# puzzlepaint/surfelmeshing

Hardware: AMD Instinct MI355X
Metric: RGB-D frames/s integrated @640x480, 5M live surfels; achieved HBM GB/s (higher is better)
Workload: dtype f32; 1 GPU; C2: synthetic room stream 640x480, raw depth + colour frames resident in HBM, full preprocessing + Integrate per frame, 4912850 live surfels (6250000 slots), steady-state re-traversal; max_surfel_count=6250000, streams=1, parallelism=1 independent stream per GPU

## Files before the change

### surfelmeshing_amd/csrc/smx_recon.hip

```cpp
#include <math.h>
#include <cmath>
#include <stdlib.h>
#include <string.h>

#include <algorithm>
#include <atomic>
#include <vector>

#include "smx_recon_state.hpp"
#include "smx_mesh.hpp"
#include <hip/hip_ext.h>

using namespace smx;

namespace {

struct FrameCtx {
  Mat34 L;
  Mat34 G;
  float fx, fy, cx, cy;
  Unproj up;
  float inv_depth_scaling;
  float sensor_noise_factor;
  float cos_normal_compat;
// ... 462 lines not shown
    return __builtin_amdgcn_readfirstlane(longest) * kSubLists;
  }
  ent = 0; cntv = 0;
  return (n_slots_scan + kBlock - 1) / kBlock;
}
template <bool kUseList>
__device__ __forceinline__ bool vis_entry(uint32_t ent, uint32_t c, uint32_t cntv, uint32_t n_slots_scan, uint32_t lane, uint32_t& i) {
  if (kUseList) {
    const uint32_t k = __builtin_amdgcn_readfirstlane(c % kSubLists);
    const uint32_t len = (uint32_t)__builtin_amdgcn_readlane((int)cntv, (int)k);
    i = ent;
    return (c / kSubLists) * (uint32_t)kBlock + lane < len;
  }
  i = c * kBlock + lane;
  return i < n_slots_scan;
}

struct PairRec { uint32_t i, code; Vec3 g, l, gn; float r2; };
__device__ __forceinline__ PairRec fetch_pair(const Surfels& S, const FrameCtx& c, uint32_t i, uint32_t code) {
  const float4 p4 = *S.group(kGroupP, i), n4 = *S.group(kGroupN, i);
  PairRec r;
  r.i = i; r.code = code;
  r.g = Vec3{p4.x, p4.y, p4.z};
  r.l = mul(c.L, r.g);
  r.gn = Vec3{n4.x, n4.y, n4.z};
  r.r2 = n4.w;
  return r;
}
struct TileLds {
  int zmin[kTilePx];
  uint32_t sup[kTilePx], cnt[kTilePx], confl[kTilePx];
  unsigned long long sum[kTilePx];
  float2 nrm[kTilePx];
  uint16_t depth[kTilePx];
};
__device__ __forceinline__ void assoc_stage(TileLds& t, const FrameCtx& c, const PairRec& r) {
  if (!(r.code & kPairActive)) return;
  const uint32_t k = r.code & 255u;
  const float measurement_depth = c.inv_depth_scaling * (float)t.depth[k];
  if (measurement_depth <= 0) return;
  const float first = __int_as_float(t.zmin[k]);
  if (first < (1 - c.sensor_noise_factor) * measurement_depth) {
    if (first == r.l.z) atomicMin(&t.confl[k], 0x80000000u | r.i);
    return;
  }
  const float occlusion_depth = (1 + c.sensor_noise_factor) * measurement_depth;
  if (r.l.z > occlusion_depth) return;
  const float surfel_distance = sqrtf(r.l.x * r.l.x + r.l.y * r.l.y + r.l.z * r.l.z);
  const Vec3 ln = rotate(c.L, r.gn);
  const float dot_angle = (1.0f / surfel_distance) * (r.l.x * ln.x + r.l.y * ln.y + r.l.z * ln.z);
  if (dot_angle > 0) return;
  if (measurement_depth < r.l.z) {
    const float2 n = t.nrm[k];
    const float nz = meas_normal_z(n.x, n.y);
    const float d = ln.x * n.x + ln.y * n.y + ln.z * nz;
    if (d < c.cos_normal_compat) return;
  }
  if (r.r2 <= 0) return;
  atomicMin(&t.sup[k], r.i);
  atomicAdd(&t.cnt[k], 1u);
  atomicAdd(&t.sum[k], (unsigned long long)q_from_float(r.l.z));
}
__device__ __forceinline__ uint32_t merge_candidate(TileLds& t, const FrameCtx& c, const PairRec& r) {
  if (r.code & kPairSecond) return kInvalid;
  if (!(r.r2 >= 0)) return kInvalid;
  const uint32_t k = r.code & 255u;
// ... 28 lines not shown
  const float dx = r.g.x - sp4.x, dy = r.g.y - sp4.y, dz = r.g.z - sp4.z;
  const float d2 = dx * dx + dy * dy + dz * dz;
  const float kDist = 0.5f * (0.25f * 0.25f);
  if (d2 > kDist * (r.r2 + other_r2)) return;
  const float dot_angle = r.gn.x * sn4.x + r.gn.y * sn4.y + r.gn.z * sn4.z;
  if (dot_angle < 0.93969f) return;
  merge_flag[r.i] = 1;
}
__device__ __forceinline__ void merge_stage(TileLds& t, const Surfels& S, const FrameCtx& c, const PairRec& r,
                                            uint8_t* __restrict__ merge_flag) {
  const uint32_t s = merge_candidate(t, c, r);
  if (s == kInvalid) return;
  const float4 sp4 = *S.group(kGroupP, s), sn4 = *S.group(kGroupN, s);
  keep(sp4); keep(sn4);
  merge_decide(r, sp4, sn4, merge_flag);
}

constexpr int kPairCache = 4;
template <class F>
__device__ __forceinline__ void for_uncached_pairs(const Surfels& S, const FrameCtx& c, const TileBins& tb, uint32_t tile,
                                                   uint32_t n_binned, bool overflowed, uint32_t n_ovf, F f) {
  for (uint32_t k = kPairCache * kTilePx + threadIdx.x; k < n_binned; k += kTilePx) {
    const uint2 pr = tb.pairs[(size_t)tile * tb.cap + k];
    f(fetch_pair(S, c, pr.x, pr.y));
  }
  if (overflowed)
    for (uint32_t e = threadIdx.x; e < n_ovf; e += kTilePx) {
      const uint4 o = tb.ovf[e];
      if (o.x == tile) f(fetch_pair(S, c, o.y, o.z));
    }
}

__global__ void __launch_bounds__(kTilePx)
k_assoc_tiles(Surfels S, FrameCtx c, Scratch sc, Img<const uint16_t> depth, Img<const float2> normals, TileBins tb,
              uint32_t* __restrict__ next_ovf_count, uint8_t* __restrict__ merge_flag, DevState* st,
              const uint8_t* __restrict__ seg_act, uint32_t nseg, uint32_t* __restrict__ direction_out, uint32_t* __restrict__ seg_work_count,
              unsigned long long* stamps, const unsigned long long* __restrict__ ts_ring, volatile unsigned long long* ts_host,
              unsigned long long ts_seq) {
  SMX_SET_WAVE_PRIO();
  __shared__ TileLds t;
  __shared__ uint32_t order_wave_tot[kTilePx / 64];
  ts_begin(c.ts, kTsTilesBegin);
  if (blockIdx.x == 0 && threadIdx.x == 64 && ts_host && ts_seq > 2) {
    const unsigned long long q = ts_seq - 2;
    const unsigned long long* src = ts_ring + (size_t)(q % kTsRing) * kTsWords;
    volatile unsigned long long* dst = ts_host + (size_t)(q % kTsRing) * kTsWords;
    unsigned long long w[kTsWords];
#pragma unroll
    for (int k = 0; k < kTsWords; ++k) w[k] = src[k];
    if (w[kTsSeq] == q) {
      unsigned long long check = q ^ kTsCheckSalt;
#pragma unroll
      for (int k = 1; k < kTsSeqTail; ++k) check ^= w[k];
      dst[kTsSeq] = q;
#pragma unroll
      for (int k = 1; k < kTsSeqTail; ++k) dst[k] = w[k];
      dst[kTsSeqTail] = check;
    }
  }
  if (blockIdx.x == 0) {
    const uint32_t n_used = min(nseg, (st->surfel_count + (uint32_t)kSeg - 1u) / (uint32_t)kSeg);
    choose_segment_direction(seg_act, n_used, direction_out, order_wave_tot);
    __syncthreads();
  }
  SMX_STAMP(stamps, 0);
  const uint32_t tile = blockIdx.x, lane = threadIdx.x;
  const int x = (int)(tile % (uint32_t)tb.tiles_x) * kTileW + (int)(lane % kTileW);
  const int y = (int)(tile / (uint32_t)tb.tiles_x) * kTileH + (int)(lane / kTileW);
  const bool in_image = x < c.W && y < c.H;
  const uint32_t n_total = tb.count[tile * kCountStride];
  const uint32_t n_ovf = *tb.ovf_count;
  const uint32_t n_binned = n_total < tb.cap ? n_total : tb.cap;
  const bool overflowed = n_total > tb.cap;
  uint2 pr[kPairCache];
  bool have[kPairCache];
#pragma unroll
  for (int q = 0; q < kPairCache; ++q) {
    const uint32_t k = q * kTilePx + lane;
    have[q] = k < n_binned;
    pr[q] = tb.pairs[(size_t)tile * tb.cap + (have[q] ? k : 0u)];
  }
#pragma unroll
  for (int q = 0; q < kPairCache; ++q) { keep(pr[q].x); keep(pr[q].y); if (!have[q]) pr[q] = make_uint2(0u, 0u); }
  const uint16_t own_depth = in_image ? depth(y, x) : (uint16_t)0;
  const float2 own_normal = in_image ? normals(y, x) : make_float2(0.f, 0.f);
  PairRec rec[kPairCache];
#pragma unroll
  for (int q = 0; q < kPairCache; ++q) rec[q] = fetch_pair(S, c, pr[q].x, pr[q].y);
  t.zmin[lane] = 0x7F800000;
  t.sup[lane] = kInvalid; t.cnt[lane] = 0; t.confl[lane] = kInvalid; t.sum[lane] = 0;
  t.depth[lane] = own_depth; t.nrm[lane] = own_normal;
  __syncthreads();
  SMX_STAMP(stamps, 1);
  auto zmin_stage = [&](const PairRec& r) { if (r.code & kPairActive) atomicMin(&t.zmin[r.code & 255u], __float_as_int(r.l.z)); };
#pragma unroll
  for (int q = 0; q < kPairCache; ++q) if (have[q]) zmin_stage(rec[q]);
  for_uncached_pairs(S, c, tb, tile, n_binned, overflowed, n_ovf, zmin_stage);
  __syncthreads();
  SMX_STAMP(stamps, 2);
  if (lane == 0) {
    tb.count[tile * kCountStride] = 0;
    if (tile == 0) { *next_ovf_count = 0; seg_work_count[0] = 0; seg_work_count[1] = 0; }
    if (c.stats) {
      atomicAdd(&st->n_pairs, n_total);
      atomicMax(&st->max_tile_pairs, n_total);
      if (tile == 0) st->n_overflow_pairs = n_ovf;
    }
  }
#pragma unroll
  for (int q = 0; q < kPairCache; ++q) if (have[q]) assoc_stage(t, c, rec[q]);
  for_uncached_pairs(S, c, tb, tile, n_binned, overflowed, n_ovf, [&](const PairRec& r) { assoc_stage(t, c, r); });
  __syncthreads();
  SMX_STAMP(stamps, 3);
  uint32_t cand[kPairCache];
  float4 cp4[kPairCache], cn4[kPairCache];
#pragma unroll
  for (int q = 0; q < kPairCache; ++q) cand[q] = have[q] ? merge_candidate(t, c, rec[q]) : kInvalid;
#pragma unroll
  for (int q = 0; q < kPairCache; ++q) {
    const uint32_t g = cand[q] == kInvalid ? 0u : cand[q];
    cp4[q] = *S.group(kGroupP, g); cn4[q] = *S.group(kGroupN, g);
  }
#pragma unroll
  for (int q = 0; q < kPairCache; ++q) { keep(cp4[q]); keep(cn4[q]); }
#pragma unroll
  for (int q = 0; q < kPairCache; ++q) if (cand[q] != kInvalid) merge_decide(rec[q], cp4[q], cn4[q], merge_flag);
  for_uncached_pairs(S, c, tb, tile, n_binned, overflowed, n_ovf, [&](const PairRec& r) { merge_stage(t, S, c, r, merge_flag); });
  __syncthreads();
  SMX_STAMP(stamps, 4);
  if (in_image) {
    const size_t k = (size_t)y * c.W + x;
    sc.first_depth[k] = __int_as_float(t.zmin[lane]);
    sc.supporting[k] = t.sup[lane];
    sc.counts[k] = t.cnt[lane];
    sc.depth_sums[k] = (long long)t.sum[lane];
    sc.confl_key[k] = t.confl[lane];
  }
  SMX_STAMP(stamps, 5);
  ts_end(c.ts, kTsTilesEnd, blockIdx.x, gridDim.x);
}

__device__ __forceinline__ float depth_sum_avg(const Scratch& sc, size_t k) {
  return q_to_float(sc.depth_sums[k]) / (float)sc.counts[k];
}

__global__ void __launch_bounds__(kBlock)
k_blend_start(float ds, Img<uint16_t> depth, Scratch sc, BlendBufs b, int W, int H, unsigned long long* ts) {
  ts_end(ts, kTsBlendEnd, blockIdx.y * gridDim.x + blockIdx.x, gridDim.x * gridDim.y);
  const int x = blockIdx.x * 64 + (threadIdx.x & 63);
  const int y = blockIdx.y * 4 + (threadIdx.x >> 6);
  if (!(x >= 1 && y >= 1 && x < W - 1 && y < H - 1)) return;
  const size_t k = (size_t)y * W + x;
  const uint16_t own = depth(y, x);
  if (own == 0 || sc.supporting[k] == kInvalid) return;
  bool measurement_border = false, surfel_border = false;
  for (int wy = y - 1; wy <= y + 1; ++wy)
    for (int wx = x - 1; wx <= x + 1; ++wx) {
      if (depth(wy, wx) == 0) measurement_border = true;
      else if (sc.supporting[(size_t)wy * W + wx] == kInvalid) surfel_border = true;
    }
  if (surfel_border) {
    b.new_distance_map[k] = 1;
    const float avg = depth_sum_avg(sc, k);
    b.new_deltas[k] = avg - (float)own / ds;
  }
  if (measurement_border) {
    b.distance_map[k] = 1;
    const float avg = depth_sum_avg(sc, k);
    b.deltas[k] = avg - (float)own / ds;
// ... 318 lines not shown
  for (int off = 1; off < 64; off <<= 1) {
    const uint32_t t = __shfl_up(incl, off);
    if (lane >= (uint32_t)off) incl += t;
  }
  if (lane == 63) wave_tot[wave] = incl;
  __syncthreads();
  uint32_t wave_off = 0, total = 0;
#pragma unroll
  for (int w = 0; w < kBlock / 64; ++w) {
    if ((uint32_t)w < wave) wave_off += wave_tot[w];
    total += wave_tot[w];
  }
  uint32_t run = wave_off + incl - mine;
#pragma unroll
  for (int j = 0; j < kScanPxPerThread; ++j) {
    const int k = k0 + j;
    if (k < P) local_rank[k] = run;
    run += f[j];
  }
  if (threadIdx.x == 0) {
    block_sums[block] = total;
    if (block == 0) st->create_base_next = st->surfel_count;
  }
}

struct FrameIn {
  Img<const uint16_t> depth; Img<const float2> normals; Img<const float> radius; Img<const uchar3> color;
};

struct PixelIn {
  uint16_t depth; float first; uint32_t key; uint32_t count; float2 nxy; uchar3 col; float radius;
};
__device__ __forceinline__ PixelIn load_pixel(const FrameCtx& c, const Scratch& sc, const FrameIn& in, int x, int y) {
  const size_t k = (size_t)y * c.W + x;
  PixelIn p;
  p.depth = in.depth(y, x); p.first = sc.first_depth[k]; p.key = sc.confl_key[k]; p.count = sc.counts[k];
  p.nxy = in.normals(y, x); p.col = in.color(y, x); p.radius = in.radius(y, x);
  return p;
}

__device__ __forceinline__ void keep(const PixelIn& p) {
  keep((uint32_t)p.depth); keep(p.first); keep(p.key); keep(p.count); keep(p.nxy); keep(p.radius);
  keep((uint32_t)p.col.x | ((uint32_t)p.col.y << 8) | ((uint32_t)p.col.z << 16));
}

struct SurfelRegs {
  float4 P;
  float4 N;
  float4 C;
  bool dirty;
  bool replaced;
  Vec3 new_smooth;
};

__device__ __forceinline__ void integrate_or_conflict(SurfelRegs& R, const FrameCtx& c, const PixelIn& px,
                                                      bool integrate, int x, int y,
                                                      const Vec3& cam, uint32_t i, DevState* st) {
  if (!integrate) return;
  const float measurement_depth = c.inv_depth_scaling * (float)px.depth;
  if (measurement_depth <= 0) return;
  bool conflicting = false;
  const float first = px.first;
  if (first < (1 - c.sensor_noise_factor) * measurement_depth) {
    if (first == cam.z) {
      const uint32_t key = px.key;
      if (key != kInvalid && (key & 0x7FFFFFFFu) == i) conflicting = true;
    }
    integrate = false;
  }
  if (!integrate && !conflicting) return;
// ... 259 lines not shown
      if (j < per && bidx < n_scan_blocks) { block_offsets[bidx] = run; run += v[j]; }
    }
  } else {
    for (int j = 0; j < per; ++j) {
      const int bidx = threadIdx.x * per + j;
      if (bidx < n_scan_blocks) mine += block_sums[bidx];
    }
    uint32_t run = block_excl_scan(mine, wave_tot, total);
    for (int j = 0; j < per; ++j) {
      const int bidx = threadIdx.x * per + j;
      if (bidx < n_scan_blocks) { block_offsets[bidx] = run; run += block_sums[bidx]; }
    }
  }
  __syncthreads();
  const uint32_t room = max_surfels - base;
  const uint32_t created = total < room ? total : room;
  if (block == 0) {
    for (int bidx = threadIdx.x; bidx < n_scan_blocks; bidx += kBlock) block_offsets_out[bidx] = block_offsets[bidx];
    if (threadIdx.x == 0) {
      st->create_base = base;
      st->new_count = created;
      st->capacity_clamped = (total > room) ? 1u : 0u;
      st->surfel_count = base + created;
    }
  }
  const int kDX[4] = {-1, 1, 0, 0}, kDY[4] = {0, 0, -1, 1};
  const int W = c.W, H = c.H, P = W * H;
  for (int k = block * kBlock + threadIdx.x; k < P; k += n_blocks * kBlock) {
    const uint32_t rank = block_offsets[k / kScanPxPerBlock] + ranks[k];
    if (flags[k] != 1 || rank >= created) continue;
    const int y = k / W, x = k - y * W;
    const uint32_t i = base + rank;
    const uint32_t depth_u = in.depth(y, x);
    const float2 nxy = in.normals(y, x);
    const uchar3 col = in.color(y, x);
    const float r2 = in.radius(y, x);
    uint32_t nsup[4], nflag[4], nrank_local[4], ndepth_u[4];
    int kks[4];
#pragma unroll
    for (int d = 0; d < 4; ++d) {
      const int yy = min(max(y + kDY[d], 0), H - 1), xx = min(max(x + kDX[d], 0), W - 1);
      kks[d] = yy * W + xx;
      nsup[d] = sc.supporting[kks[d]];
      nflag[d] = flags[kks[d]];
      nrank_local[d] = ranks[kks[d]];
      ndepth_u[d] = in.depth(yy, xx);
    }
    keep(depth_u); keep(nxy); keep(r2); keep((uint32_t)col.x | ((uint32_t)col.y << 8) | ((uint32_t)col.z << 16));
#pragma unroll
    for (int d = 0; d < 4; ++d) { keep(nsup[d]); keep(nflag[d]); keep(nrank_local[d]); keep(ndepth_u[d]); }
    float4 np4[4], ns4[4];
#pragma unroll
    for (int d = 0; d < 4; ++d) {
      const uint32_t gidx = nsup[d] != kInvalid ? nsup[d] : base;
      np4[d] = *S.group(kGroupP, gidx);
      ns4[d] = *S.group(kGroupS, gidx);
    }
#pragma unroll
    for (int d = 0; d < 4; ++d) { keep(np4[d]); keep(ns4[d]); }
    const float depth = c.inv_depth_scaling * (float)depth_u;
    const Vec3 lp = {depth * (c.up.fx_inv * (float)x + c.up.cx_inv), depth * (c.up.fy_inv * (float)y + c.up.cy_inv), depth};
    const Vec3 gp = mul(c.G, lp);
    const Vec3 mn = {nxy.x, nxy.y, meas_normal_z(nxy.x, nxy.y)};
    const Vec3 gn = rotate(c.G, mn);
    Vec3 sum = {0, 0, 0};
    int count_plus_1 = 1;
    uint32_t nbs[4];
#pragma unroll
    for (int d = 0; d < 4; ++d) {
      uint32_t nb = nsup[d];
      if (nb != kInvalid) {
        const float dx = np4[d].x - gp.x, dy = np4[d].y - gp.y, dz = np4[d].z - gp.z;
        const float d2 = dx * dx + dy * dy + dz * dz;
        if (d2 > c.rf2 * r2) nb = kInvalid;
        else {
          sum.x = sum.x + ns4[d].x; sum.y = sum.y + ns4[d].y; sum.z = sum.z + ns4[d].z;
          ++count_plus_1;
        }
      } else if (nflag[d] == 1) {
        const uint32_t nrank = block_offsets[kks[d] / kScanPxPerBlock] + nrank_local[d];
        if (nrank < created) {
// ... 679 lines not shown
  }
  if (threadIdx.x == 0) *total_out = carry;
}
__global__ void __launch_bounds__(kBlock)
k_delta_gather(Surfels S, uint8_t* __restrict__ dirty8, const uint32_t* __restrict__ seg_offset, float* __restrict__ out,
               uint32_t total, const DevState* st) {
  __shared__ uint32_t wave_tot[kBlock / 64];
  const uint32_t N = st->surfel_count, i0 = blockIdx.x * kSeg + threadIdx.x * 4;
  uint32_t bits = 0;
  if (i0 < N) {
    const uchar4 d = *reinterpret_cast<const uchar4*>(&dirty8[i0]);
    bits = (d.x != 0 ? 1u : 0u) | ((i0 + 1 < N && d.y != 0) ? 2u : 0u) | ((i0 + 2 < N && d.z != 0) ? 4u : 0u) |
           ((i0 + 3 < N && d.w != 0) ? 8u : 0u);
    if (bits) *reinterpret_cast<uchar4*>(&dirty8[i0]) = make_uchar4(0, 0, 0, 0);
  }
  uint32_t seg_total;
  uint32_t off = seg_offset[blockIdx.x] + block_excl_scan((uint32_t)__popc(bits), wave_tot, seg_total);
  const int want[8] = {kSmoothX, kSmoothY, kSmoothZ, kRadiusSq, kNormalX, kNormalY, kNormalZ, kLastUpdateStamp};
#pragma unroll
  for (int j = 0; j < 4; ++j)
    if (bits & (1u << j)) {
      const uint32_t i = i0 + j;
      out[off] = __uint_as_float(i);
#pragma unroll
      for (int k = 0; k < 8; ++k) out[(size_t)(k + 1) * total + off] = S.f(want[k], i);
      ++off;
    }
}

__global__ void __launch_bounds__(kBlock)
k_decode_conflicting(const uint32_t* __restrict__ key, uint32_t* __restrict__ out, int P) {
  const int k = blockIdx.x * kBlock + threadIdx.x;
  if (k < P) out[k] = (key[k] == kInvalid) ? kInvalid : (key[k] & 0x7FFFFFFFu);
}

__global__ void __launch_bounds__(kBlock)
k_global_ranks(const uint32_t* __restrict__ local_rank, const uint32_t* __restrict__ block_offsets,
               uint32_t* __restrict__ out, int P) {
  const int k = blockIdx.x * kBlock + threadIdx.x;
  if (k < P) out[k] = block_offsets[k / kScanPxPerBlock] + local_rank[k];
}

}

enum : int {
  kSlotScanVisible = 0, kSlotAssocTiles, kSlotBlend, kSlotIntegrate,
  kSlotUpdateNeighbors, kSlotNeighborScan,
  kSlotRegAccumulate, kSlotRegStep,
  kSlotRegUpdate,
  kSlotCull,
  kSlotEmpty,
  kSlotCount
};
static const char* const kSlotNames[kSlotCount] = {
  "scan_visible", "assoc_tiles", "blend", "integrate+new_flags", "update_neighbors+create",
  "neighbor_scan", "reg_accumulate", "reg_step", "reg_update", "cull_segments", "empty_slot"};

struct SlotTimer {
  smx_recon r; hipStream_t st; int slot; bool kev, prof, by_launch;
  SlotTimer(smx_recon r_, hipStream_t st_, int slot_, bool launch_carries = false) : r(r_), st(st_), slot(slot_) {
    kev = (r->timing_enabled & 2) != 0;
    prof = (r->prof_slot == slot) && r->prof_ev && r->prof_n < r->prof_cap;
    by_launch = prof && launch_carries;
    if (kev) (void)hipEventRecord(r->kev[2 * slot], st);
    if (prof && !by_launch) (void)hipEventRecord(r->prof_ev[2 * r->prof_n], st);
  }
// ... 162 lines not shown
  r->L.rec_chunks.stride = (uint32_t)(div_up(r->nsegB, kSubLists) + 8192);
  SMX_TRY(r->mem.alloc(&r->L.rec_chunks.desc, (size_t)kSubLists * r->L.rec_chunks.stride, true));
  SMX_TRY(r->mem.alloc(&r->L.rec_chunks.count, (size_t)kSubLists * kCountStride, true));
  static_assert(kSegAcc == kSegB && kAccCount < kCountStride, "pass B lists the edge kernel's segments by its own segment numbers");
  r->L.acc_chunks.stride = r->L.rec_chunks.stride;
  r->L.acc_chunks.count = r->L.rec_chunks.count + kAccCount;
  SMX_TRY(r->mem.alloc(&r->L.acc_chunks.desc, (size_t)kSubLists * r->L.acc_chunks.stride, true));
  SMX_TRY(r->mem.alloc(&r->flags_buf[0], (size_t)r->nsegB * kSegB, true));
  SMX_TRY(r->mem.alloc(&r->flags_buf[1], (size_t)r->nsegB * kSegB, true));
  r->L.flags8 = r->flags_buf[0];
  r->L.hot_shift = 10;
  while ((((size_t)r->nseg * kSeg) >> r->L.hot_shift) + 1 > (size_t)kMaxHotGroups) ++r->L.hot_shift;
  r->L.n_hot_groups = (uint32_t)((((size_t)r->nseg * kSeg) >> r->L.hot_shift) + 1);
  SMX_TRY(r->mem.alloc(&r->L.hot_epoch, (size_t)r->L.n_hot_groups + 64, true));
  SMX_TRY(r->mem.alloc(&r->L.seg_targets, (size_t)r->nsegB * kBlockB, true));
  r->L.epoch = 128;
  r->hot_filter_enabled = 1;
  r->fuse_edges = kFuseEdgesDefault;
  r->hot_holdoff = 3;
  SMX_TRY(r->mem.alloc(&r->merge_flag, r->S.pitch, true));
  SMX_TRY(r->mem.alloc(&r->gate_count, 32, true));
  r->gate_expected = 0;
  constexpr int kHandoverModeDefault = 1;
  r->handover_mode = kHandoverModeDefault;
  {
    const char* cc = getenv("ROCPROF_COUNTER_COLLECTION");
    if (cc && cc[0] && strcmp(cc, "0") != 0) r->handover_mode = 0;
  }
  SMX_TRY(r->mem.alloc(&r->L.act_list, (size_t)r->nsegB * kSegB, true));
  SMX_TRY(r->mem.alloc(&r->sc.supporting, P, true));
  SMX_TRY(r->mem.alloc(&r->sc.counts, P, true));
  SMX_TRY(r->mem.alloc(&r->sc.depth_sums, P, true));
  SMX_TRY(r->mem.alloc(&r->sc.confl_key, P, true));
  SMX_TRY(r->mem.alloc(&r->sc.first_depth, P, true));
  for (int k = 0; k < 2; ++k) {
    SMX_TRY(r->mem.alloc(&r->vis_count_set[k], (size_t)kSubLists * kCountStride, true));
    SMX_TRY(r->mem.alloc(&r->ovf_count_set[k], 1, true));
  }
  r->L.vis_chunks.count = r->vis_count_set[0];
  r->tb.tiles_x = div_up(width, kTileW);
  r->tb.n_tiles = (uint32_t)(r->tb.tiles_x * div_up(height, kTileH));
  r->tb.cap = r->bin_cap_full = kTileBinCap;
  SMX_TRY(r->mem.alloc(&r->tb.pairs, (size_t)r->tb.n_tiles * kTileBinCap, false));
  SMX_TRY(r->mem.alloc(&r->tb.count, (size_t)r->tb.n_tiles * kCountStride, true));
  SMX_TRY(r->mem.alloc(&r->tb.ovf, 2 * (size_t)r->S.pitch + 64, false));
  r->tb.ovf_count = r->ovf_count_set[0];
#ifdef SMX_STAMPS
  SMX_TRY(r->mem.alloc(&r->stamps, (size_t)3 * 16 * 8192, true));
#endif
  SMX_TRY(r->mem.alloc(&r->blended_depth, P, true));
  SMX_TRY(r->mem.alloc(&r->bb.distance_map, P, true));
  SMX_TRY(r->mem.alloc(&r->bb.new_distance_map, P, true));
  SMX_TRY(r->mem.alloc(&r->bb.deltas, P, true));
  SMX_TRY(r->mem.alloc(&r->bb.new_deltas, P, true));
  SMX_TRY(r->mem.alloc(&r->new_flags, P, true));
  SMX_TRY(r->mem.alloc(&r->new_ranks, P, true));
  SMX_TRY(r->mem.alloc(&r->tmp_u32, P, true));
  r->n_scan_blocks = div_up((long long)P, kScanPxPerBlock);
  SMX_TRY(r->mem.alloc(&r->block_sums, (size_t)r->n_scan_blocks, true));
  SMX_TRY(r->mem.alloc(&r->block_offsets, (size_t)r->n_scan_blocks, true));
  SMX_TRY(r->mem.alloc(&r->st, 1, true));
  SMX_TRY(r->mem.alloc(&r->ts_ring, (size_t)kTsRing * kTsWords, true));
  SMX_TRY(r->mem.alloc_host(&r->ts_host, (size_t)kTsRing * kTsWords, false));
  SMX_TRY(r->mem.alloc_host(&r->ts_mapped, (size_t)kTsRing * kTsWords, true));
  memset(const_cast<unsigned long long*>(r->ts_mapped), 0, sizeof(unsigned long long) * kTsRing * kTsWords);
  SMX_TRY(hip_rc(hipHostGetDevicePointer(reinterpret_cast<void**>(&r->ts_mapped_dev), const_cast<unsigned long long*>(r->ts_mapped), 0), "hipHostGetDevicePointer"));
  SMX_TRY(hip_rc(hipDeviceGetAttribute(&r->wall_khz, hipDeviceAttributeWallClockRate, device), "hipDeviceGetAttribute"));
// ... 189 lines not shown
  const Img<uint16_t> depth_rw = as_img<uint16_t>(depth);

  const uint8_t* flags_prev = r->L.flags8;
  r->L.flags8 = (r->L.flags8 == r->flags_buf[0]) ? r->flags_buf[1] : r->flags_buf[0];
  r->L.epoch = (r->L.epoch + 1u) & 255u;
  if (r->hot_holdoff > 0) --r->hot_holdoff;
  const bool pipelined = r->overlap_enabled != 0;
  const hipStream_t sF = st;
  const hipStream_t sR = pipelined ? r->reg_stream : st;
  const bool split = pipelined && (r->debug_skip & 16) != 0;
  if (r->reg_pending && r->last_stream != st) SMX_CALL(join_regularizer(r, st));
  r->last_stream = st;
  if (r->stats_enabled) hipLaunchKernelGGL(k_reset_frame_stats, dim3(1), dim3(1), 0, sF, r->st, 1);
  if (tm) SMX_HIP(hipEventRecord(r->ev[0], sF));
  r->L.descending = *reinterpret_cast<volatile uint32_t*>(r->dir_host);
  r->sc_cur ^= 1;
  r->L.vis_chunks.count = r->vis_count_set[r->sc_cur];
  r->tb.ovf_count = r->ovf_count_set[r->sc_cur];
  if (hook_ready) SMX_HIP(hipStreamWaitEvent(sF, hook_ready, 0));
  {
    SlotTimer t(r, sF, kSlotCull);
    if (r->sw_dirty) SMX_HIP(hipMemsetAsync(r->sw.count, 0, 2 * sizeof(uint32_t), sF));
    r->sw_dirty = true;
    hipLaunchKernelGGL(k_cull_segments, dim3((unsigned)div_up(r->nseg, kBlock)), b, 0, sF, c, r->L, r->sw, r->st, (uint32_t)r->nseg, (uint32_t)P, r->ts_seq); }
  if (r->pending_mark) { SMX_HIP(hipStreamWaitEvent(sF, r->pending_mark, 0)); r->pending_mark = nullptr; }
  if (r->stats_enabled) hipLaunchKernelGGL(k_reset_frame_stats, dim3(1), dim3(1), 0, sF, r->st, 0);
  { SlotTimer t(r, sF, kSlotScanVisible, true);
    const bool lds_tables = !r->no_lds_tables;
    constexpr int kPassAWgsPerCu = 8;
    const dim3 ga((unsigned)(r->cu_count * kPassAWgsPerCu));
    hipExtLaunchKernelGGL(k_scan_visible, ga, b, 0, sF, t.start(), t.stop(), 0, r->S, c, r->L, r->tb, r->sw, flags_prev, r->st, lds_tables ? 1 : 0);
    r->table_valid = true; r->table_frame = frame_index; r->table_window = c.reg_window; }
  { SlotTimer t(r, sF, kSlotAssocTiles, true);
    hipExtLaunchKernelGGL(k_assoc_tiles, dim3(r->tb.n_tiles), dim3(kTilePx), 0, sF, t.start(), t.stop(), 0, r->S, c, r->sc, in.depth, in.normals, r->tb,
                       r->ovf_count_set[r->sc_cur ^ 1], r->merge_flag, r->st, r->L.seg_act, (uint32_t)r->nseg, r->dir_dev, r->sw.count,
                       r->stamps ? r->stamps : nullptr, r->ts_ring, c.ts ? r->ts_mapped_dev : nullptr, r->ts_seq);
    r->sw_dirty = false; }
  if (tm) { SMX_HIP(hipEventRecord(r->ev[1], sF)); SMX_HIP(hipEventRecord(r->ev[2], sF)); SMX_HIP(hipEventRecord(r->ev[3], sF)); SMX_HIP(hipEventRecord(r->ev[4], sF)); }
  const int halo = p->measurement_blending_radius - 1;
  const bool fused_blend = p->do_blending && halo <= kBlendMaxHalo && !r->blend_multi_launch;
  bool front_by_launch = false, front_by_gate = false;
  const float ds = 1.0f / c.inv_depth_scaling;
  const float term = p->do_blending ? 1.0f / ((float)p->measurement_blending_radius - 1.0f) : 0.0f;
  const Img<uint16_t> blended = {r->blended_depth, r->H, r->W, (size_t)r->W * sizeof(uint16_t)};
  if (fused_blend) {
    front_by_gate = pipelined && !split && r->handover_mode == 1 && !(r->debug_skip & 4) && !tm && !(r->timing_enabled & 2);
    SlotTimer t(r, sF, kSlotBlend, front_by_gate);
    const int cus = r->cu_count;
    int tile = 32;
    if (40 + 2 * halo <= 64) {
      auto cost = [&](int t) { const long long n = (long long)div_up(r->W, t) * div_up(r->H, t); return ((n + cus - 1) / cus) * (long long)(t + 2 * halo) * (t + 2 * halo); };
      if ((cost(40) < cost(32)) != (r->blend_other_tile != 0)) tile = 40;
    }
    const int rw = tile + 2 * halo;
    const size_t lds = sizeof(BlendMasks) + (size_t)rw * rw * 10;
    const int tiles_x = div_up(r->W, tile);
    const uint32_t n_blend = (uint32_t)(tiles_x * div_up(r->H, tile));
    unsigned long long* stamps = (r->stamps && (frame_index & 63u) == 32u) ? r->stamps + 16 * 8192 : nullptr;
    front_by_launch = !front_by_gate && pipelined && !split && !tm && !(r->timing_enabled & 2) && r->prof_slot != kSlotBlend;
    uint32_t* const gate = front_by_gate ? r->gate_count : nullptr;
    if (front_by_gate) r->gate_expected += n_blend;
    const hipEvent_t start = front_by_gate ? t.start() : nullptr;
    const hipEvent_t stop = front_by_gate ? t.stop() : front_by_launch ? r->ev_front : nullptr;
    if (tile == 40)
      hipExtLaunchKernelGGL(k_blend_tiles<40>, dim3(n_blend), dim3(kBlendThreads), (uint32_t)lds, sF, start, stop, 0, p->measurement_blending_radius, term, ds,
                            in.depth, blended, r->sc, r->W, r->H, tiles_x, stamps, c.ts, gate, (r->debug_skip & 256) ? 1 : kBlendMaxRings);
    else
// ... 289 lines not shown
  SMX_HIP(hipStreamSynchronize(st));
  d->frame_index = frame_index;
  d->surfel_count = n;
  d->count = total;
  if (total > d->capacity) {
    set_error("delta of %u slots does not fit the capacity %u", total, d->capacity);
    return SMX_ERR_INVALID_ARGUMENT;
  }
  if (total == 0) return SMX_OK;
  SMX_CHECK_ARG(d->surfel_index && d->x && d->y && d->z && d->radius_squared && d->normal_x && d->normal_y &&
                d->normal_z && d->last_update_stamp);
  SMX_CALL(acquire_staging(r, st, (size_t)9 * total));
  hipLaunchKernelGGL(k_delta_gather, dim3(r->nseg), dim3(kBlock), 0, st, r->S, r->L.dirty8, r->delta_seg.get(), r->staging.buf.get(), total,
                     r->st);
  SMX_LAUNCH_CHECK();
  void* dst[9] = {d->surfel_index, d->x, d->y, d->z, d->radius_squared, d->normal_x, d->normal_y, d->normal_z,
                  d->last_update_stamp};
  for (int k = 0; k < 9; ++k)
    SMX_HIP(hipMemcpyAsync(dst[k], r->staging.buf.get() + (size_t)k * total, (size_t)total * 4, hipMemcpyDeviceToHost, st));
  SMX_HIP(hipStreamSynchronize(st));
  return SMX_OK;
}

int smx_recon_debug_download_scratch(smx_recon r, smx_stream s, int32_t which, void* dst) {
  SMX_CHECK_ARG(r != nullptr && dst != nullptr);
  SMX_ON_DEVICE(r->device);
  SMX_CALL(join_regularizer(r, (hipStream_t)s));
  hipStream_t st = (hipStream_t)s;
  const size_t P = (size_t)r->W * r->H;
  const void* src = nullptr; size_t bytes = 0;
  switch (which) {
    case SMX_SCRATCH_SUPPORTING: src = r->sc.supporting; bytes = P * 4; break;
    case SMX_SCRATCH_SUPPORT_COUNTS: src = r->sc.counts; bytes = P * 4; break;
    case SMX_SCRATCH_DEPTH_SUMS: src = r->sc.depth_sums; bytes = P * 8; break;
    case SMX_SCRATCH_FIRST_DEPTH: src = r->sc.first_depth; bytes = P * 4; break;
    case SMX_SCRATCH_NEW_FLAGS: src = r->new_flags; bytes = P; break;
    case SMX_SCRATCH_CONFLICTING:
      hipLaunchKernelGGL(k_decode_conflicting, dim3(div_up((long long)P, kBlock)), dim3(kBlock), 0, st, r->sc.confl_key, r->tmp_u32, (int)P);
      src = r->tmp_u32; bytes = P * 4; break;
    case SMX_SCRATCH_NEW_INDICES:
      hipLaunchKernelGGL(k_global_ranks, dim3(div_up((long long)P, kBlock)), dim3(kBlock), 0, st, r->new_ranks, r->block_offsets, r->tmp_u32, (int)P);
      src = r->tmp_u32; bytes = P * 4; break;
    default: set_error("unknown scratch id %d", which); return SMX_ERR_INVALID_ARGUMENT;
  }
  SMX_HIP(hipMemcpyAsync(dst, src, bytes, hipMemcpyDeviceToHost, st));
  SMX_HIP(hipStreamSynchronize(st));
  return SMX_OK;
}

int smx_recon_debug_count_skipped_segments(smx_recon r, smx_stream s, uint32_t* out) {
  SMX_CHECK_ARG(r != nullptr && out != nullptr);
  SMX_ON_DEVICE(r->device);
  SMX_CALL(join_regularizer(r, (hipStream_t)s));
  std::vector<uint32_t> marks((size_t)r->nsegB);
  SMX_HIP(hipMemcpyAsync(marks.data(), r->L.recent_seg, marks.size() * 4, hipMemcpyDeviceToHost, (hipStream_t)s));
  SMX_HIP(hipStreamSynchronize((hipStream_t)s));
  uint32_t n = 0;
  for (uint32_t m : marks) n += m == kInvalid ? 1u : 0u;
  *out = n;
  return SMX_OK;
}

}
```

### surfelmeshing_amd/csrc/smx_recon_state.hpp

```cpp
#pragma once

#include "smx_common.hpp"
#include "smx_components.hpp"
#include "smx_decimate.hpp"
#include "smx_distance.hpp"
#include "smx_fill.hpp"
#include "smx_raycast.hpp"
#include "smx_render.hpp"
#include "smx_sample.hpp"
#include "smx_track.hpp"

namespace smx {

struct MeshWorkspace;

enum : int {
  kX = 0, kY = 1, kZ = 2, kSmoothX = 3, kSmoothY = 4, kSmoothZ = 5, kConfidence = 6, kRadiusSq = 7,
  kNormalX = 8, kNormalY = 9, kNormalZ = 10, kGradX = 11, kGradY = 12, kGradZ = 13,
  kCreationStamp = 17, kLastUpdateStamp = 18, kNeighbor0 = 19, kGradCount = 23, kColor = 24, kRows = 25
};

struct DevState {
  uint32_t surfel_count;
  uint32_t merge_count;
// ... 6 lines not shown
  uint32_t n_window_edges, n_contributors;
  uint32_t n_segments_skipped;
  uint32_t reg_saturated;
  uint32_t n_pairs, n_overflow_pairs, max_tile_pairs;
};

enum : int { kGroupP = 0, kGroupS, kGroupN, kGroupT, kGroupC, kGroupG, kGroups };
__host__ __device__ constexpr int row_group(int row) {
  return row <= 2 ? kGroupP : row <= 5 ? kGroupS : row == 6 ? kGroupC : row == 7 ? kGroupN : row <= 10 ? kGroupN
       : row <= 13 ? kGroupG : row <= 16 ? -1 : row == 17 ? kGroupC : row == 18 ? kGroupP : row <= 22 ? kGroupT
       : row == 24 ? kGroupC : -1;
}
__host__ __device__ constexpr int row_sub(int row) {
  return row <= 2 ? row : row <= 5 ? row - 3 : row == 6 ? 0 : row == 7 ? 3 : row <= 10 ? row - 8
       : row <= 13 ? row - 11 : row == 17 ? 1 : row == 18 ? 3 : row <= 22 ? row - 19 : row == 24 ? 2 : -1;
}
__host__ __device__ constexpr int group_start(int g) { return g; }
constexpr int kQuadsPerSlot = 6;
struct Surfels {
  float* base;
  size_t pitch;
  __host__ __device__ __forceinline__ size_t quad(int g, uint32_t i) const { return (size_t)group_start(g) * pitch + (size_t)i; }
  __device__ __forceinline__ float& f(int row, uint32_t i) const { return base[quad(row_group(row), i) * 4 + row_sub(row)]; }
  __device__ __forceinline__ uint32_t& u(int row, uint32_t i) const {
    return reinterpret_cast<uint32_t*>(base)[quad(row_group(row), i) * 4 + row_sub(row)];
  }
  __device__ __forceinline__ float4* group(int g, uint32_t i) const { return reinterpret_cast<float4*>(base) + quad(g, i); }
  __device__ __forceinline__ void set_neighbors(uint32_t i, const uint4& t) const { *reinterpret_cast<uint4*>(group(kGroupT, i)) = t; }
  __device__ __forceinline__ void set_neighbor(uint32_t i, int q, uint32_t v) const { u(kNeighbor0 + q, i) = v; }
  struct View { const float4* p; size_t stride; };
  View view(int g) const { return View{reinterpret_cast<const float4*>(base) + quad(g, 0), quad(g, 1) - quad(g, 0)}; }
};

struct Scratch {
  uint32_t* supporting;
  uint32_t* counts;
  long long* depth_sums;
  uint32_t* confl_key;
  float* first_depth;
};

constexpr int kBlock = 256;

inline unsigned blocks_for(uint32_t n) { return (unsigned)div_up(n, kBlock); }
inline bool finite_f(float v) { return v - v == 0.0f; }
inline bool ranges_overlap(const void* a, size_t a_bytes, const void* b, size_t b_bytes) {
  if (!a || !b || a_bytes == 0 || b_bytes == 0) return false;
  const uintptr_t a0 = (uintptr_t)a, b0 = (uintptr_t)b;
  return a0 < b0 + b_bytes && b0 < a0 + a_bytes;
}
inline unsigned long long word64(const uint32_t* h, int lo) { return ((unsigned long long)h[lo + 1] << 32) | h[lo]; }

constexpr int kSeg = 1024;
constexpr int kSegB = 1024;
constexpr int kBlockB = kSegB / 4;
constexpr uint32_t kCountStride = 32;
constexpr uint32_t kSubLists = 16;
struct Chunks { uint32_t* desc; uint32_t* count; uint32_t stride; };
struct Lists {
  Chunks vis_chunks, rec_chunks;
  Chunks acc_chunks;
  uint32_t* vis_list;
  uint32_t vis_region;
  float* seg_box;
  uint32_t* vis_seg;
  uint8_t* seg_streak;
  uint32_t* recent_list;
  uint32_t* recent_seg;
  uint32_t* act_list;
  uint8_t* flags8;
  uint8_t* dirty8;
  uint8_t* seg_act;
// ... 234 lines not shown
```

Before: 6111 frames/s.

## Pack per-pixel association results and inputs into a 32-byte record

The association tile kernel now also loads each pixel's radius and colour and writes a 32-byte per-pixel record holding first depth, conflict key, count, supporting index, normal, radius and packed colour, using two 16-byte stores. Later kernels (load_pixel and surfel creation) read this record with vector loads instead of gathering from several separate scratch and image arrays. The separate first_depth buffer is replaced by the record, and a decode kernel keeps the debug readback working. The tile kernel does more loads and stores, and the record duplicates data still written to the separate arrays, so total bytes moved may rise even though consumers issue fewer, wider accesses.

```diff
diff --git a/surfelmeshing_amd/csrc/smx_recon.hip b/surfelmeshing_amd/csrc/smx_recon.hip
--- a/surfelmeshing_amd/csrc/smx_recon.hip
+++ b/surfelmeshing_amd/csrc/smx_recon.hip
@@ -518,6 +518,7 @@
   uint32_t sup[kTilePx], cnt[kTilePx], confl[kTilePx];
   unsigned long long sum[kTilePx];
   float2 nrm[kTilePx];
+  float radius[kTilePx]; uint32_t colour[kTilePx];
   uint16_t depth[kTilePx];
 };
 __device__ __forceinline__ void assoc_stage(TileLds& t, const FrameCtx& c, const PairRec& r) {
@@ -612,7 +613,8 @@
 }
 
 __global__ void __launch_bounds__(kTilePx)
-k_assoc_tiles(Surfels S, FrameCtx c, Scratch sc, Img<const uint16_t> depth, Img<const float2> normals, TileBins tb,
+k_assoc_tiles(Surfels S, FrameCtx c, Scratch sc, Img<const uint16_t> depth, Img<const float2> normals,
+              Img<const float> radius, Img<const uchar3> color, TileBins tb,
               uint32_t* __restrict__ next_ovf_count, uint8_t* __restrict__ merge_flag, DevState* st,
               const uint8_t* __restrict__ seg_act, uint32_t nseg, uint32_t* __restrict__ direction_out, uint32_t* __restrict__ seg_work_count,
               unsigned long long* stamps, const unsigned long long* __restrict__ ts_ring, volatile unsigned long long* ts_host,
@@ -664,12 +666,16 @@
   for (int q = 0; q < kPairCache; ++q) { keep(pr[q].x); keep(pr[q].y); if (!have[q]) pr[q] = make_uint2(0u, 0u); }
   const uint16_t own_depth = in_image ? depth(y, x) : (uint16_t)0;
   const float2 own_normal = in_image ? normals(y, x) : make_float2(0.f, 0.f);
+  const float own_radius = in_image ? radius(y, x) : 0.f;
+  const uchar3 own_color = in_image ? color(y, x) : make_uchar3(0, 0, 0);
   PairRec rec[kPairCache];
 #pragma unroll
   for (int q = 0; q < kPairCache; ++q) rec[q] = fetch_pair(S, c, pr[q].x, pr[q].y);
   t.zmin[lane] = 0x7F800000;
   t.sup[lane] = kInvalid; t.cnt[lane] = 0; t.confl[lane] = kInvalid; t.sum[lane] = 0;
   t.depth[lane] = own_depth; t.nrm[lane] = own_normal;
+  t.radius[lane] = own_radius;
+  t.colour[lane] = (uint32_t)own_color.x | ((uint32_t)own_color.y << 8) | ((uint32_t)own_color.z << 16);
   __syncthreads();
   SMX_STAMP(stamps, 1);
   auto zmin_stage = [&](const PairRec& r) { if (r.code & kPairActive) atomicMin(&t.zmin[r.code & 255u], __float_as_int(r.l.z)); };
@@ -710,11 +716,16 @@
   SMX_STAMP(stamps, 4);
   if (in_image) {
     const size_t k = (size_t)y * c.W + x;
-    sc.first_depth[k] = __int_as_float(t.zmin[lane]);
-    sc.supporting[k] = t.sup[lane];
+    const uint32_t sup = t.sup[lane], confl = t.confl[lane];
+    const float2 n = t.nrm[lane];
+    PixelRec* const pr = sc.rec + k;
+    out_store16(pr, make_uint4((uint32_t)t.zmin[lane], confl, t.cnt[lane], sup));
+    out_store16(reinterpret_cast<uint4*>(pr) + 1,
+                make_uint4(__float_as_uint(n.x), __float_as_uint(n.y), __float_as_uint(t.radius[lane]), t.colour[lane]));
+    sc.supporting[k] = sup;
     sc.counts[k] = t.cnt[lane];
     sc.depth_sums[k] = (long long)t.sum[lane];
-    sc.confl_key[k] = t.confl[lane];
+    sc.confl_key[k] = confl;
   }
   SMX_STAMP(stamps, 5);
   ts_end(c.ts, kTsTilesEnd, blockIdx.x, gridDim.x);
@@ -1099,10 +1110,12 @@
   uint16_t depth; float first; uint32_t key; uint32_t count; float2 nxy; uchar3 col; float radius;
 };
 __device__ __forceinline__ PixelIn load_pixel(const FrameCtx& c, const Scratch& sc, const FrameIn& in, int x, int y) {
-  const size_t k = (size_t)y * c.W + x;
+  const uint4* const q = reinterpret_cast<const uint4*>(sc.rec + ((size_t)y * c.W + x));
+  const uint4 a = q[0], b = q[1];
   PixelIn p;
-  p.depth = in.depth(y, x); p.first = sc.first_depth[k]; p.key = sc.confl_key[k]; p.count = sc.counts[k];
-  p.nxy = in.normals(y, x); p.col = in.color(y, x); p.radius = in.radius(y, x);
+  p.depth = in.depth(y, x); p.first = __uint_as_float(a.x); p.key = a.y; p.count = a.z;
+  p.nxy = make_float2(__uint_as_float(b.x), __uint_as_float(b.y)); p.radius = __uint_as_float(b.z);
+  p.col = make_uchar3((unsigned char)b.w, (unsigned char)(b.w >> 8), (unsigned char)(b.w >> 16));
   return p;
 }
 
@@ -1428,9 +1441,10 @@
     const int y = k / W, x = k - y * W;
     const uint32_t i = base + rank;
     const uint32_t depth_u = in.depth(y, x);
-    const float2 nxy = in.normals(y, x);
-    const uchar3 col = in.color(y, x);
-    const float r2 = in.radius(y, x);
+    const uint4 own = reinterpret_cast<const uint4*>(sc.rec + k)[1];
+    const float2 nxy = make_float2(__uint_as_float(own.x), __uint_as_float(own.y));
+    const uchar3 col = make_uchar3((unsigned char)own.w, (unsigned char)(own.w >> 8), (unsigned char)(own.w >> 16));
+    const float r2 = __uint_as_float(own.z);
     uint32_t nsup[4], nflag[4], nrank_local[4], ndepth_u[4];
     int kks[4];
 #pragma unroll
@@ -1442,7 +1456,7 @@
       nrank_local[d] = ranks[kks[d]];
       ndepth_u[d] = in.depth(yy, xx);
     }
-    keep(depth_u); keep(nxy); keep(r2); keep((uint32_t)col.x | ((uint32_t)col.y << 8) | ((uint32_t)col.z << 16));
+    keep(depth_u); keep(own);
 #pragma unroll
     for (int d = 0; d < 4; ++d) { keep(nsup[d]); keep(nflag[d]); keep(nrank_local[d]); keep(ndepth_u[d]); }
     float4 np4[4], ns4[4];
@@ -2188,6 +2202,12 @@
 k_decode_conflicting(const uint32_t* __restrict__ key, uint32_t* __restrict__ out, int P) {
   const int k = blockIdx.x * kBlock + threadIdx.x;
   if (k < P) out[k] = (key[k] == kInvalid) ? kInvalid : (key[k] & 0x7FFFFFFFu);
+}
+
+__global__ void __launch_bounds__(kBlock)
+k_decode_first_depth(const PixelRec* __restrict__ rec, uint32_t* __restrict__ out, int P) {
+  const int k = blockIdx.x * kBlock + threadIdx.x;
+  if (k < P) out[k] = __float_as_uint(rec[k].first_depth);
 }
 
 __global__ void __launch_bounds__(kBlock)
@@ -2416,7 +2436,7 @@
   SMX_TRY(r->mem.alloc(&r->sc.counts, P, true));
   SMX_TRY(r->mem.alloc(&r->sc.depth_sums, P, true));
   SMX_TRY(r->mem.alloc(&r->sc.confl_key, P, true));
-  SMX_TRY(r->mem.alloc(&r->sc.first_depth, P, true));
+  SMX_TRY(r->mem.alloc(&r->sc.rec, P, true));
   for (int k = 0; k < 2; ++k) {
     SMX_TRY(r->mem.alloc(&r->vis_count_set[k], (size_t)kSubLists * kCountStride, true));
     SMX_TRY(r->mem.alloc(&r->ovf_count_set[k], 1, true));
@@ -2672,7 +2692,7 @@
     hipExtLaunchKernelGGL(k_scan_visible, ga, b, 0, sF, t.start(), t.stop(), 0, r->S, c, r->L, r->tb, r->sw, flags_prev, r->st, lds_tables ? 1 : 0);
     r->table_valid = true; r->table_frame = frame_index; r->table_window = c.reg_window; }
   { SlotTimer t(r, sF, kSlotAssocTiles, true);
-    hipExtLaunchKernelGGL(k_assoc_tiles, dim3(r->tb.n_tiles), dim3(kTilePx), 0, sF, t.start(), t.stop(), 0, r->S, c, r->sc, in.depth, in.normals, r->tb,
+    hipExtLaunchKernelGGL(k_assoc_tiles, dim3(r->tb.n_tiles), dim3(kTilePx), 0, sF, t.start(), t.stop(), 0, r->S, c, r->sc, in.depth, in.normals, in.radius, in.color, r->tb,
                        r->ovf_count_set[r->sc_cur ^ 1], r->merge_flag, r->st, r->L.seg_act, (uint32_t)r->nseg, r->dir_dev, r->sw.count,
                        r->stamps ? r->stamps : nullptr, r->ts_ring, c.ts ? r->ts_mapped_dev : nullptr, r->ts_seq);
     r->sw_dirty = false; }
@@ -3028,8 +3048,10 @@
   switch (which) {
     case SMX_SCRATCH_SUPPORTING: src = r->sc.supporting; bytes = P * 4; break;
     case SMX_SCRATCH_SUPPORT_COUNTS: src = r->sc.counts; bytes = P * 4; break;
+    case SMX_SCRATCH_FIRST_DEPTH:
+      hipLaunchKernelGGL(k_decode_first_depth, dim3(div_up((long long)P, kBlock)), dim3(kBlock), 0, st, r->sc.rec, r->tmp_u32, (int)P);
+      src = r->tmp_u32; bytes = P * 4; break;
     case SMX_SCRATCH_DEPTH_SUMS: src = r->sc.depth_sums; bytes = P * 8; break;
-    case SMX_SCRATCH_FIRST_DEPTH: src = r->sc.first_depth; bytes = P * 4; break;
     case SMX_SCRATCH_NEW_FLAGS: src = r->new_flags; bytes = P; break;
     case SMX_SCRATCH_CONFLICTING:
       hipLaunchKernelGGL(k_decode_conflicting, dim3(div_up((long long)P, kBlock)), dim3(kBlock), 0, st, r->sc.confl_key, r->tmp_u32, (int)P);
diff --git a/surfelmeshing_amd/csrc/smx_recon_state.hpp b/surfelmeshing_amd/csrc/smx_recon_state.hpp
--- a/surfelmeshing_amd/csrc/smx_recon_state.hpp
+++ b/surfelmeshing_amd/csrc/smx_recon_state.hpp
@@ -62,12 +62,22 @@
   View view(int g) const { return View{reinterpret_cast<const float4*>(base) + quad(g, 0), quad(g, 1) - quad(g, 0)}; }
 };
 
+struct alignas(32) PixelRec {
+  float first_depth;
+  uint32_t confl_key;
+  uint32_t counts;
+  uint32_t supporting;
+  float nx, ny;
+  float radius;
+  uint32_t colour;
+};
+static_assert(sizeof(PixelRec) == 32, "two 16-byte halves");
 struct Scratch {
   uint32_t* supporting;
   uint32_t* counts;
   long long* depth_sums;
   uint32_t* confl_key;
-  float* first_depth;
+  PixelRec* rec;
 };
 
 constexpr int kBlock = 256;
```

Result: no change. 6158 frames/s, median of 6 (+0.8%).
